# unanan/UNet_Nested4Tiny_Objects_Keypoints

Hardware: AMD Instinct MI355X
Metric: images/sec (train step) UNet++ L=4 256x256 (higher is better)
Workload: dtype f32

## Files before the change

include/unetpp_hip.h:

```cpp
#ifndef UNETPP_HIP_H
#define UNETPP_HIP_H

#include <stdint.h>

#ifdef __cplusplus
extern "C" {
#endif

#define UNETPP_ABI_VERSION 12
#define UNETPP_MAX_VIEWS 8

#define UNETPP_OK 0
#define UNETPP_EINVAL (-1)
#define UNETPP_ELAUNCH (-2)

typedef struct unetpp_view {
  float* ptr;
  int32_t C, c_off, c_len;
  int32_t Hs, Ws;
  int32_t sy, sx, oy, ox;
  const float* scale;
  const float* shift;
  const float* gate;
  int32_t relu;
// ... 207 lines not shown
                         float* out_nchw, void* stream);
int unetpp_head_bwd_bf16(const float* d_out_nchw, const float* out_nchw, const void* x, const float* weight,
                         int32_t N, int32_t H, int32_t W, int32_t C, int32_t n_cls, float p_drop, uint64_t seed,
                         const uint8_t* mask, const uint64_t* seed_dev, void* dx, int32_t accumulate, int32_t gate_x, float* partial,
                         void* stream);

int unetpp_maxpool_bwd_bf16(const void* d_pooled, const uint8_t* pool_idx, int32_t N, int32_t H, int32_t W, int32_t C,
                            void* d_act, const void* gate, void* stream);
int unetpp_bilinear2x_fwd_bf16(const void* x, int32_t N, int32_t H, int32_t W, int32_t C, void* y, void* stream);
int unetpp_bilinear2x_bwd_bf16(const void* dy, int32_t N, int32_t H, int32_t W, int32_t C, void* dx, int32_t accumulate,
                               const void* gate, void* stream);

int unetpp_first_layer_dgrad_bf16(const void* dy, const float* weight, int32_t N, int32_t H, int32_t W, int32_t CIN,
                                  int32_t COUT, float* dx, void* stream);

int64_t unetpp_heatmap_pattern_workspace_bytes(int32_t N, int32_t n_maps, int32_t H, int32_t W);
int unetpp_heatmap_pattern(const float* points, int32_t N, int32_t P, const int32_t* map_points,
                           const int32_t* map_begin, int32_t n_maps, int32_t H, int32_t W, float radius,
                           float* out_nchw, void* workspace, void* stream);
int64_t unetpp_keypoints_workspace_bytes(int32_t maps, int32_t H, int32_t W, int32_t max_regions);
int unetpp_keypoints_extract(int32_t stage, const float* heat, int32_t maps, int32_t H, int32_t W,
                             const float* thr_per_map, int32_t num, int32_t max_regions, int32_t sweeps,
                             void* workspace, int32_t* changed, float* points, int32_t* counts, void* stream);

#define UNETPP_OPTIM_ADAMW 0
#define UNETPP_OPTIM_ADABOUND 1
#define UNETPP_OPTIM_SGDW 2
#define UNETPP_OPTIM_AMS 1
#define UNETPP_OPTIM_CAPTURABLE 2
#define UNETPP_OPTIM_HYPER 8
// ... 125 lines not shown
```

unet_nested4tiny_objects_keypoints_amd/_lib.py:

```python
from __future__ import annotations

import ctypes as C
import os
import subprocess

_PKG_DIR = os.path.dirname(os.path.abspath(__file__))
_REPO = os.path.dirname(_PKG_DIR)
LIB_PATH = os.environ.get("UNETPP_LIB", os.path.join(_PKG_DIR, "libunetpp_hip.so"))
CSRC = os.path.join(_PKG_DIR, "csrc")
INCLUDE = os.path.join(_REPO, "include")
SOURCES = ("gemm_pix.hip", "gemm_fast.hip", "gemm_pw.hip", "gemm_pw_bf16.hip", "gemm_wino.hip", "gemm_bf16.hip", "gemm_bf16_dma.hip", "wgrad_bf16.hip", "pointwise_bf16.hip", "keypoints.hip", "weight_image.hip", "wgrad.hip", "wgrad_fast.hip", "wgrad_dma.hip", "wgrad_pw.hip", "wgrad_wino.hip", "first_layer.hip", "pointwise.hip", "caller.hip", "optim.hip", "validate.hip", "average.hip", "loader.hip", "scene.hip",
           "detect.hip", "crops.hip", "topk_loss.hip")
HEADERS = ("common.h", "gemm_units.h", "wgrad_reduce.h", "lds_asm.h", "bf16_common.h", "dropout.h", "bn_fused.h",
           "wino_experiments.h", "dma_experiments.h", "heads_mean.h", "focal_element.h")
MAX_VIEWS = 8
ABI_VERSION = 12
EXTRA_FLAGS = {"gemm_wino.hip": ("-fno-slp-vectorize",), "wgrad_wino.hip": ("-fno-slp-vectorize",)}
GEMM_DIRECT = 1
GEMM_BF16 = 2


class View(C.Structure):
    _fields_ = [
        ("ptr", C.c_void_p),
        ("C", C.c_int32), ("c_off", C.c_int32), ("c_len", C.c_int32),
        ("Hs", C.c_int32), ("Ws", C.c_int32),
        ("sy", C.c_int32), ("sx", C.c_int32), ("oy", C.c_int32), ("ox", C.c_int32),
        ("scale", C.c_void_p), ("shift", C.c_void_p), ("gate", C.c_void_p),
        ("relu", C.c_int32), ("accumulate", C.c_int32), ("gate_sum", C.c_int32), ("reserved", C.c_int32),
    ]


class BnFused(C.Structure):
    _fields_ = [
# ... 199 lines not shown
    "unetpp_optim_step_clip": (C.c_int, [_I32, _I32, _P, _I32, _P, _I64, _P, _P, _P, _P, _P, _P]),
    "unetpp_grad_scale": (C.c_int, [_P, _I32, _P, _I64, _P, _F, _P, _P]),
    "unetpp_warp_batch": (C.c_int, [_P, _I32, _I64, _I32, _I32, _I32, _P, _I32, _P, _P, _P, _F, _P, _I32, _I32, _P, _I32,
                                    _P, _P, _P]),
    "unetpp_augment_draw": (C.c_int, [_P, _I32, _U64, _I32, _I32, _I32, _I32, C.POINTER(AugmentDesc), _P]),
    "unetpp_scene_stitch": (C.c_int, [_P, _I32, _I32, _I32, _I32, _I32, C.POINTER(C.c_int32), C.POINTER(SceneRect), _P, _P,
                                      _I32, _I32, _I32, _P]),
    "unetpp_peaks_workspace_bytes": (_I64, [_I32, _I32, _I32]),
    "unetpp_peaks_detect": (C.c_int, [_P, _I32, _I32, _I32, _F, _I32, _I32, _I32, _P, _P, _P, _P, _P]),
    "unetpp_detect_match": (C.c_int, [_P, _P, _P, _I32, _I32, _I32, _P, _P, _I32, _F, _P, _P, _P, _P]),
    "unetpp_points_target": (C.c_int, [_P, _P, _I64, _I32, _P, _I32, _P, _I32, _I32, _I32, _F, _P, _P]),
    "unetpp_crops_draw": (C.c_int, [_P, _P, _P, _I32, _U64, _I32, _I32, _I32, _I32, _I32, _P, _P, _I32, _F, _F, _F,
                                    C.POINTER(AugmentDesc), _P]),
    "unetpp_topk_focal_workspace_bytes": (_I64, [_I32, _I64, _I64]),
    "unetpp_topk_focal_heads": (C.c_int, [C.POINTER(FocalHeads), _P, _I64, _I64, _I64, _I64, _F, _P, _P, _P, _P]),
}

_LIB = None


def source_hash() -> str:
    import hashlib
    h = hashlib.sha256()
    for path in [os.path.join(CSRC, s) for s in SOURCES + HEADERS] + [os.path.join(INCLUDE, "unetpp_hip.h")]:
        with open(path, "rb") as f:
            h.update(f.read())
    return h.hexdigest()[:16]


def build_library(force: bool = False, verbose: bool = False, out_path: str = None, obj_dir: str = None) -> str:
# ... 75 lines not shown
```

unet_nested4tiny_objects_keypoints_amd/csrc/common.h:

```cpp
#pragma once
#include <hip/hip_runtime.h>
#include <stdint.h>

#include "unetpp_hip.h"

typedef float f32x16 __attribute__((ext_vector_type(16)));
typedef float f32x4 __attribute__((ext_vector_type(4)));

namespace unetpp {

constexpr int kBlockPixels = 256;
constexpr int kThreads = 256;
constexpr int kMaxHaloPixels = 340;

struct TileGeom {
  int log2tw, tiles_x, tiles_y;
};

inline TileGeom tile_geom(int H, int W) {
  int l = 3;
  while ((1 << l) < W && l < 5) ++l;
  TileGeom g;
  g.log2tw = l;
  const int TW = 1 << l, TH = kBlockPixels >> l;
// ... 104 lines not shown
  OPT_BF16_DMA_MIN8,
  OPT_BF16_DMA_FORM,
  OPT_BF16_DMA_SMALL,
  OPT_BF16_DMA_STATS,
  OPT_BF16_DMA_POINTWISE,
  OPT_BF16_DMA_SPLIT,
  OPT_BF16_WGRAD_QUAD,
  OPT_WINO_NO_LEAN,
  OPT_WINO_ONE_PER_CU,
  OPT_MEMSET_NODES,
  OPT_BF16_PW_PLAIN,
  OPT_PW_DIRECT,
  OPT_PW_NT,
  OPT_HEAD_WGS_PER_CU,
  OPT_SMALL_WGRAD_BLOCKS,
  OPT_COUNT
};
bool opt_is_set(Opt o);
long opt_value(Opt o, long dflt);

int launch_gemm_fast(const unetpp_gemm_desc* d, hipStream_t st);
int launch_gemm_pw(const unetpp_gemm_desc* d, const struct FastArgs& fa, hipStream_t st);
int launch_gemm_pw_bf16(const unetpp_gemm_desc* d, const struct FastArgs& fa, hipStream_t st);
bool wino_applies(const unetpp_gemm_desc* d);
int launch_gemm_wino(const unetpp_gemm_desc* d, hipStream_t st, long* bn_rows);
bool bf16_gemm_args(const unetpp_gemm_desc* d, struct FastArgs& a);
int launch_gemm_bf16(const unetpp_gemm_desc* d, hipStream_t st);
int launch_gemm_bf16_dma(const unetpp_gemm_desc* d, hipStream_t st);
enum WgradKernel {
  WGRAD_FIRST_LAYER, WGRAD_BF16_QUAD, WGRAD_BF16_PAIR, WGRAD_PW, WGRAD_WINO, WGRAD_DMA, WGRAD_FAST, WGRAD_GENERIC
// ... 30 lines not shown
```

unet_nested4tiny_objects_keypoints_amd/csrc/first_layer.hip:

```cpp
#include "bf16_common.h"
#include "bn_fused.h"
#include "common.h"
#include "lds_asm.h"

namespace unetpp {
namespace {

constexpr int kMaxCout = 128;

struct SmallArgs {
  const float* x;
  const float* w;
  const float* bias;
  float* y;
  const float* dy;
  float* stats;
  float* slabs;
  int N, H, W, COUT, yC, relu;
  int log2tw, tiles_x, tiles_y;
  long n_patches;
  int bn_in_kernel;
};

template <int CIN>
__device__ __forceinline__ void stage_patch(const SmallArgs& a, float* xs, int n, int ty0, int tx0, int TW, int TH) {
  const int HWp = TW + 2, npix = HWp * (TH + 2);
  for (int it = threadIdx.x; it < npix * CIN; it += kThreads) {
    const int hp = it / CIN, ci = it - hp * CIN;
    const int hy = hp / HWp, hx = hp - hy * HWp;
    const int y = ty0 + hy - 1, x = tx0 + hx - 1;
    float v = 0.f;
    if (y >= 0 && y < a.H && x >= 0 && x < a.W) v = a.x[((static_cast<long>(n) * a.H + y) * a.W + x) * CIN + ci];
    xs[it] = v;
  }
}

template <int CIN, bool BF = false>
__global__ __launch_bounds__(kThreads, CIN >= 3 ? 3 : 4) void small_cin_fwd_kernel(const SmallArgs a) {
  constexpr int ITEMS = (kMaxHaloPixels * CIN + kThreads - 1) / kThreads;
  constexpr bool WREG = CIN <= 3;
  __shared__ float xs2[2][kMaxHaloPixels * CIN];
  __shared__ __attribute__((aligned(16))) float ws[WREG ? 4 : 9 * CIN * kMaxCout];
  __shared__ float red[4][kMaxCout * 2];
  const int tid = threadIdx.x;
  const bool bn_fused = a.bn_in_kernel != 0;
  float run1 = 0.f, run2 = 0.f;
  const int TW = 1 << a.log2tw, TH = kBlockPixels >> a.log2tw, HWp = TW + 2;
  const int npix = HWp * (TH + 2);
  const int QN = a.COUT >> 2;
// ... 46 lines not shown
    if (patch + gridDim.x < n_patches) request(patch + gridDim.x);

    unsigned b = patch;
    const int txi = static_cast<int>(b % static_cast<unsigned>(a.tiles_x));
    b /= static_cast<unsigned>(a.tiles_x);
    const int tyi = static_cast<int>(b % static_cast<unsigned>(a.tiles_y));
    const int n = static_cast<int>(b / static_cast<unsigned>(a.tiles_y));
    const int ty0 = tyi * TH, tx0 = txi * TW;
    float* y_patch = BF ? reinterpret_cast<float*>(reinterpret_cast<bf16_t*>(a.y) + ((static_cast<long>(n) * a.H + ty0) * a.W + tx0) * a.yC)
                        : a.y + ((static_cast<long>(n) * a.H + ty0) * a.W + tx0) * a.yC;
    f32x2_t s1a = {0.f, 0.f}, s1b = {0.f, 0.f}, s2a = {0.f, 0.f}, s2b = {0.f, 0.f};
    for (int p = psub; p < kBlockPixels; p += pstep) {
      const int py = p >> a.log2tw, px = p & (TW - 1);
      const int y = ty0 + py, x = tx0 + px;
      if (y < a.H && x < a.W) {
        f32x2_t acc_a = {bias4[0], bias4[1]}, acc_b = {bias4[2], bias4[3]};
#pragma unroll
        for (int tap = 0; tap < 9; ++tap) {
          const float* xp = &xs[((py + tap / 3) * HWp + px + tap % 3) * CIN];
#pragma unroll
          for (int ci = 0; ci < CIN; ++ci) {
            const f32x2_t xv = {xp[ci], xp[ci]};
            const f32x4 w4 = WREG ? wr[WREG ? tap * CIN + ci : 0]
                                  : *reinterpret_cast<const f32x4*>(&ws[WREG ? 0 : (tap * CIN + ci) * a.COUT + 4 * quad]);
            acc_a = __builtin_elementwise_fma(xv, f32x2_t{w4[0], w4[1]}, acc_a);
            acc_b = __builtin_elementwise_fma(xv, f32x2_t{w4[2], w4[3]}, acc_b);
          }
        }
        f32x4 acc = {acc_a.x, acc_a.y, acc_b.x, acc_b.y};
        if (a.relu) {
#pragma unroll
          for (int e = 0; e < 4; ++e) acc[e] = fmaxf(acc[e], 0.f);
        }
        if (BF) {
#pragma unroll
          for (int e = 0; e < 4; ++e) acc[e] = bf_round(acc[e]);
        }
        const f32x2_t va = {acc[0], acc[1]}, vb = {acc[2], acc[3]};
        s1a += va;
        s1b += vb;
        s2a = __builtin_elementwise_fma(va, va, s2a);
        s2b = __builtin_elementwise_fma(vb, vb, s2b);
        const unsigned o = static_cast<unsigned>((py * a.W + px) * a.yC + 4 * quad);
#ifndef UNETPP_FIRST_NO_NT
// ... 42 lines not shown
      }
    }
  }
  if (bn_fused) {
    __syncthreads();
    float* run = &red[0][0];
    if (tid < a.COUT) {
      run[2 * tid] = run1;
      run[2 * tid + 1] = run2;
    }
    __syncthreads();
    bn_rows_store<kThreads>(a.stats, a.COUT, run);
  }
}

template <int CIN, bool BF = false>
__global__ __launch_bounds__(kThreads) void small_cin_wgrad_kernel(const SmallArgs a) {
  __shared__ float xs[kMaxHaloPixels * CIN];
  __shared__ float red[kThreads][4];
  const int tid = threadIdx.x;
  const int TW = 1 << a.log2tw, TH = kBlockPixels >> a.log2tw, HWp = TW + 2;
  const int QN = a.COUT >> 2;
  const int quad = tid % QN, psub = tid / QN, pstep = kThreads / QN;
  f32x4 acc[9 * CIN];
#pragma unroll
  for (int i = 0; i < 9 * CIN; ++i) acc[i] = f32x4{0.f, 0.f, 0.f, 0.f};
  f32x4 db = {0.f, 0.f, 0.f, 0.f};
  for (long patch = blockIdx.x; patch < a.n_patches; patch += gridDim.x) {
    long b = patch;
    const int txi = static_cast<int>(b % a.tiles_x);
// ... 32 lines not shown
#pragma unroll
        for (int e = 0; e < 4; ++e) db[e] += g[e];
#pragma unroll
        for (int tap = 0; tap < 9; ++tap) {
          const float* xp = &xs[((py + tap / 3) * HWp + px + tap % 3) * CIN];
#pragma unroll
          for (int ci = 0; ci < CIN; ++ci) {
            const float xv = xp[ci];
#pragma unroll
            for (int e = 0; e < 4; ++e) acc[tap * CIN + ci][e] = fmaf(xv, g[e], acc[tap * CIN + ci][e]);
          }
        }
      }
    }
  }
  float* slab = a.slabs + static_cast<long>(blockIdx.x) * (9 * CIN + 1) * a.COUT;
#pragma unroll
  for (int row = 0; row <= 9 * CIN; ++row) {
    const f32x4 v = (row < 9 * CIN) ? acc[row < 9 * CIN ? row : 0] : db;
    __syncthreads();
#pragma unroll
    for (int e = 0; e < 4; ++e) red[tid][e] = v[e];
    __syncthreads();
    for (int c = tid; c < a.COUT; c += kThreads) {
      const int q = c >> 2, e = c & 3;
      float t = 0.f;
      for (int k = q; k < kThreads; k += QN) t += red[k][e];
      slab[row * a.COUT + c] = t;
    }
  }
}

template <int CIN>
__global__ __launch_bounds__(kThreads) void small_cin_dgrad_bf16_kernel(const bf16_t* __restrict__ dy,
                                                                        const float* __restrict__ w, int N, int H, int W,
                                                                        int COUT, float* __restrict__ dx) {
  __shared__ float ws[9 * kMaxCout * CIN];
  for (int i = threadIdx.x; i < 9 * COUT * CIN; i += kThreads) {
    const int ci = i % CIN, co = (i / CIN) % COUT, tap = i / (CIN * COUT);
    ws[i] = w[(static_cast<long>(co) * CIN + ci) * 9 + tap];
  }
  __syncthreads();
  const long pixels = static_cast<long>(N) * H * W;
  for (long p = blockIdx.x * static_cast<long>(kThreads) + threadIdx.x; p < pixels; p += static_cast<long>(gridDim.x) * kThreads) {
    const int x = static_cast<int>(p % W);
// ... 136 lines not shown
  if (reinterpret_cast<uintptr_t>(dy) & 15) return UNETPP_EINVAL;
  const long pixels = static_cast<long>(N) * H * W;
  long blocks = (pixels + kThreads - 1) / kThreads;
  if (blocks > 4096) blocks = 4096;
  const dim3 grid(static_cast<unsigned>(blocks)), block(kThreads);
  hipStream_t st = static_cast<hipStream_t>(stream);
  const bf16_t* g = static_cast<const bf16_t*>(dy);
  switch (CIN) {
    case 1: hipLaunchKernelGGL(small_cin_dgrad_bf16_kernel<1>, grid, block, 0, st, g, weight, N, H, W, COUT, dx); break;
    case 2: hipLaunchKernelGGL(small_cin_dgrad_bf16_kernel<2>, grid, block, 0, st, g, weight, N, H, W, COUT, dx); break;
    case 3: hipLaunchKernelGGL(small_cin_dgrad_bf16_kernel<3>, grid, block, 0, st, g, weight, N, H, W, COUT, dx); break;
    default: hipLaunchKernelGGL(small_cin_dgrad_bf16_kernel<4>, grid, block, 0, st, g, weight, N, H, W, COUT, dx); break;
  }
  return launch_status();
}
```

unet_nested4tiny_objects_keypoints_amd/csrc/gemm_pix.hip:

```cpp
#include "bn_fused.h"
#include <atomic>
#include <cstdio>
#include <cstdlib>
#include <cstring>
#include <mutex>

#include "common.h"
#include "gemm_units.h"

namespace unetpp {
namespace {

constexpr int KC = 16;
constexpr int KCP = 20;
constexpr int WJ = 12;

struct GemmArgs {
  unetpp_gemm_desc d;
  int log2tw, tiles_x, tiles_y;
  int Ktot, Ncols;
};

template <int TAPS>
__global__ __launch_bounds__(kThreads, 2) void gemm_pix_kernel(const GemmArgs a) {
// ... 138 lines not shown
      dst[1] = t2;
    }
  }
}

}
}

namespace unetpp {
namespace {
thread_local const char* g_last_kernel = "";

const char* const kOptNames[OPT_COUNT] = {
    "BF16_NO_DMA", "BF16_DMA_ALL", "BF16_DMA_MIN8", "BF16_DMA_FORM", "BF16_DMA_SMALL", "BF16_DMA_STATS",
    "BF16_DMA_POINTWISE", "BF16_DMA_SPLIT", "BF16_WGRAD_QUAD", "WINO_NO_LEAN", "WINO_ONE_PER_CU", "MEMSET_NODES",
    "BF16_PW_PLAIN", "PW_DIRECT", "PW_NT", "HEAD_WGS_PER_CU", "SMALL_WGRAD_BLOCKS"};
struct OptSlot {
  std::atomic<long> value{0};
  std::atomic<bool> set{false};
};
OptSlot g_opts[OPT_COUNT];
std::atomic<int> g_reserved_cus{0};
std::once_flag g_opts_once;

void opts_from_environment() {
  std::call_once(g_opts_once, [] {
    char name[64];
    for (int i = 0; i < OPT_COUNT; ++i) {
      snprintf(name, sizeof(name), "UNETPP_%s", kOptNames[i]);
      const char* e = getenv(name);
      if (e != nullptr) {
// ... 167 lines not shown
```

unet_nested4tiny_objects_keypoints_amd/engine.py:

```python
from __future__ import annotations

import os

from typing import Dict, List, Optional, Tuple

import torch

from . import ops
from .ops import V


USE_PACK_PLAN = os.environ.get("UNETPP_NO_PACK_PLAN") is None
USE_GROUPED_DGRAD = os.environ.get("UNETPP_NO_GROUPED_DGRAD") is None
USE_PLAN_COPIES = os.environ.get("UNETPP_NO_PLAN_COPIES") is None
_A1_MATERIALIZE_BYTES = int(float(os.environ.get("UNETPP_BF16_A1_MAX_MB", "80")) * (1 << 20))
_A1_MATERIALIZE_BYTES_F32 = int(float(os.environ.get("UNETPP_F32_A1_MAX_MB", "80")) * (1 << 20))


def _empty(n, like):
    return torch.empty(n, dtype=torch.float32, device=like.device)


def _packed(w, t, k, n, dstr, sstr, flip=False):
    dst = _empty(t * k * n, w)
    ops.pack_weight(dst, w, t, k, n, dstr, sstr, flip=flip)
    return dst


# ... 39 lines not shown
        dst, ready = plan.copy_for(("bias4", b.data_ptr()) + ops.phase_tag(plan.phase), plan.phase, (b.data_ptr(), co),
                                   lambda: (_empty(4 * co, b), [b], [(b, 0, 0, 4, co, 0, co)]))
        if ready:
            return dst
    else:
        dst = _empty(4 * co, b)
    ops.pack_weight(dst, b, 4, 1, co, (co, 0, 1), (0, 0, 1))
    return dst


def _phase_views(t, **kw):
    return [V(t, sy=2, sx=2, oy=a, ox=b, **kw) for a in (0, 1) for b in (0, 1)]


class _PairRec:
    __slots__ = ("ins", "y1", "a1", "y2", "out", "pooled", "pool_idx", "bn1", "bn2", "frozen1", "frozen2", "h", "w")

    def __init__(self):
        for s in self.__slots__:
            setattr(self, s, None)


class _UpRec:
    __slots__ = ("src", "up", "interp", "h", "w")

    def __init__(self):
        for s in self.__slots__:
            setattr(self, s, None)


class _Saved:
# ... 30 lines not shown
    conv1, conv2 = getattr(blk.conv1, "0"), getattr(blk.conv2, "0")
    co = conv1.out_channels
    like = ins[0].t
    new = lambda: torch.empty((b, h, w, co), dtype=adt, device=like.device)
    r = _PairRec()
    r.ins, r.h, r.w = ins, h, w
    if pool:
        r.pooled = torch.empty((b, h // 2, w // 2, co), dtype=adt, device=like.device)
        r.pool_idx = torch.empty((b, h // 2, w // 2, co), dtype=torch.uint8, device=like.device)
    if blk.is_batchnorm:
        bn1, bn2 = getattr(blk.conv1, "1"), getattr(blk.conv2, "1")
        t1, t2 = bool(getattr(bn1, "training", training)), bool(getattr(bn2, "training", training))
        r.frozen1, r.frozen2 = not t1, not t2
        r.y1 = new()
        r.bn1 = _conv_bn_fwd(ins, conv1, bn1, r.y1, b, h, w, t1, stats)
        r.y2 = new()
        if ((adt == torch.bfloat16 and r.y1.numel() * 2 <= _A1_MATERIALIZE_BYTES) or
                (adt == torch.float32 and r.y1.numel() * 4 <= _A1_MATERIALIZE_BYTES_F32)):
            r.a1 = new()
            ops.affine_relu_pool(r.y1, r.bn1[2], r.bn1[3], True, r.a1, None, None)
            r.bn2 = _conv_bn_fwd([V(r.a1)], conv2, bn2, r.y2, b, h, w, t2, stats)
        else:
            r.bn2 = _conv_bn_fwd([V(r.y1, scale=r.bn1[2], shift=r.bn1[3], relu=True)], conv2, bn2, r.y2, b, h, w, t2, stats)
        r.out = new()
        ops.affine_relu_pool(r.y2, r.bn2[2], r.bn2[3], True, r.out, r.pooled, r.pool_idx)
    else:
        r.a1 = new()
        ops.gemm_fwd(b, h, w, 9, ins, [V(r.a1, relu=True)], pack_conv_fwd(conv1.weight.detach()), conv1.bias.detach())
        r.out = new()
        ops.gemm_fwd(b, h, w, 9, [V(r.a1)], [V(r.out, relu=True)], pack_conv_fwd(conv2.weight.detach()),
# ... 275 lines not shown
    conv1, conv2 = getattr(blk.conv1, "0"), getattr(blk.conv2, "0")
    h, w = r.h, r.w
    if blk.is_batchnorm:
        bn1, bn2 = getattr(blk.conv1, "1"), getattr(blk.conv2, "1")
        grads[bn2.weight], grads[bn2.bias] = _bn_bwd(bn2, r.bn2, r.frozen2, d_out, r.y2, pool_grad)
        dy2 = V(d_out)
        mean, invstd, scale, shift = r.bn1
        if r.a1 is not None:
            _conv_wgrad(conv2, [V(r.a1)], [dy2], b, h, w, grads)
        else:
            _conv_wgrad(conv2, [V(r.y1, scale=scale, shift=shift, relu=True)], [dy2], b, h, w, grads)
        if flush is not None:
            flush()
        d_a1 = torch.empty_like(r.y1)
        ops.gemm_fwd(b, h, w, 9, [dy2], [V(d_a1)], pack_conv_dgrad(conv2.weight.detach()))
        grads[bn1.weight], grads[bn1.bias] = _bn_bwd(bn1, r.bn1, r.frozen1, d_a1, r.y1, None)
        dy1 = V(d_a1)
    else:
        dy2 = V(d_out) if pre_gated else V(d_out, gate=r.out)
        _conv_wgrad(conv2, [V(r.a1)], [dy2], b, h, w, grads)
        if flush is not None:
            flush()
        d_a1 = torch.empty_like(r.a1)
        ops.gemm_fwd(b, h, w, 9, [dy2], [V(d_a1, gate=r.a1)], pack_conv_dgrad(conv2.weight.detach()))
        dy1 = V(d_a1)
    _conv_wgrad(conv1, r.ins, [dy1], b, h, w, grads)
    if flush is not None:
        flush()
    if in_targets is not None:
        if dy1.t.dtype == torch.bfloat16 and in_targets[0].t.dtype == torch.float32:
# ... 207 lines not shown
```

unet_nested4tiny_objects_keypoints_amd/ops.py:

```python
from __future__ import annotations

import ctypes as C
import functools
import os
from dataclasses import dataclass
from typing import Optional, Sequence

import torch

from . import _lib
from ._lib import MAX_VIEWS, GemmDesc, PackJob, View, WeightSrc, WgradDesc, check


def _stream():
    return C.c_void_p(torch.cuda.current_stream().cuda_stream)


class LaunchTimer:

    def __init__(self):
        self.launches = []
        self.regions = []
        self.want_launches = True
        self.want_regions = True
# ... 305 lines not shown

_PLAN: Optional[PackPlan] = None


def set_pack_plan(plan: Optional[PackPlan]) -> None:
    global _PLAN
    _PLAN = plan


def current_plan() -> Optional[PackPlan]:
    return _PLAN if (_PLAN is not None and _PLAN.phase is not None) else None


def phase_tag(phase) -> tuple:
    return () if phase in ("fwd", "bwd") else (phase,)


def gemm_pixel_blocks(n: int, h: int, w: int) -> int:
    return int(_lib.lib().unetpp_gemm_pixel_blocks(n, h, w))


@dataclass
class BatchNormFinish:
    gamma: torch.Tensor
    beta: torch.Tensor
    running_mean: Optional[torch.Tensor]
    running_var: Optional[torch.Tensor]
    eps: float
    momentum: float
    count: int
# ... 213 lines not shown
                                       c, _ptr(partial), st), "unetpp_bn_bwd_reduce")
    else:
        d_pooled, pool_idx = _need(pool[0], "d_pooled"), _need(pool[1], "pool_idx", torch.uint8)
        check(lib.unetpp_bn_bwd_reduce_pool(_ptr(d_act), _ptr(y), _ptr(scale), _ptr(shift), _ptr(mean), _ptr(invstd),
                                            _ptr(d_pooled), _ptr(pool_idx), n, h, w, c, _ptr(partial), st),
              "unetpp_bn_bwd_reduce_pool")
    check(lib.unetpp_bn_bwd_finalize(_ptr(partial), blocks, c, _ptr(dgamma), _ptr(dbeta), st), "unetpp_bn_bwd_finalize")
    if pool is None:
        check(lib.unetpp_bn_bwd_apply(_ptr(d_act), _ptr(y), _ptr(scale), _ptr(shift), _ptr(mean), _ptr(invstd),
                                      _ptr(gamma), _ptr(dgamma), _ptr(dbeta), pixels, c, _ptr(dy_out), st),
              "unetpp_bn_bwd_apply")
    else:
        check(lib.unetpp_bn_bwd_apply_pool(_ptr(d_act), _ptr(y), _ptr(scale), _ptr(shift), _ptr(mean), _ptr(invstd),
                                           _ptr(gamma), _ptr(dgamma), _ptr(dbeta), _ptr(pool[0]), _ptr(pool[1]), n, h,
                                           w, c, _ptr(dy_out), st), "unetpp_bn_bwd_apply_pool")
    return dgamma, dbeta


def bn_frozen_backward(d_act, y, scale, shift, mean, invstd, dy_out, dgamma=None, dbeta=None, pool=None, want_sums=True):
    lib = _lib.lib()
    n, h, w, c = y.shape
    pixels = n * h * w
    bf16 = _is_bf16(y)
    adt = torch.bfloat16 if bf16 else torch.float32
    _need(d_act, "d_act", adt), _need(y, "y", adt), _need(dy_out, "dy", adt)
    if tuple(d_act.shape) != tuple(y.shape) or tuple(dy_out.shape) != tuple(y.shape):
        raise ValueError("d_act, y and dy must have one shape")
    if want_sums and (mean is None or invstd is None):
        raise ValueError("the gamma / beta sums need the running mean snapshot and invstd")
    blocks_fn = lib.unetpp_bn_frozen_bwd_blocks_bf16 if bf16 else lib.unetpp_bn_frozen_bwd_blocks
# ... 571 lines not shown
```

Measured before the change: 1712.

## Fuse first-layer BatchNorm backward into weight-gradient kernel with optional conv recompute

```diff
diff --git a/include/unetpp_hip.h b/include/unetpp_hip.h
--- a/include/unetpp_hip.h
+++ b/include/unetpp_hip.h
@@ -245,6 +245,20 @@
 int unetpp_first_layer_dgrad_bf16(const void* dy, const float* weight, int32_t N, int32_t H, int32_t W, int32_t CIN,
                                   int32_t COUT, float* dx, void* stream);
 
+#define UNETPP_FIRST_BN_BF16 1
+#define UNETPP_FIRST_BN_FROZEN 2
+#define UNETPP_FIRST_BN_WANT_DX 4
+#define UNETPP_FIRST_BN_UNALIGNED 8
+int unetpp_first_bn_bwd_ok(int32_t N, int32_t H, int32_t W, int32_t CIN, int32_t COUT, int32_t flags);
+int unetpp_first_bn_recomputes(int32_t CIN);
+int unetpp_first_bn_reduce(const float* x, const float* weight, const float* bias, const float* d_act, const float* y,
+                           const float* scale, const float* shift, const float* mean, const float* invstd, int32_t N,
+                           int32_t H, int32_t W, int32_t CIN, int32_t COUT, int32_t n_rows, float* partial, void* stream);
+int unetpp_first_bn_wgrad(const float* x, const float* weight, const float* bias, const float* d_act, const float* y,
+                          const float* scale, const float* shift, const float* mean, const float* invstd,
+                          const float* gamma, const float* dgamma, const float* dbeta, int32_t N, int32_t H, int32_t W,
+                          int32_t CIN, int32_t COUT, int32_t n_split, float* slabs, void* stream);
+
 int64_t unetpp_heatmap_pattern_workspace_bytes(int32_t N, int32_t n_maps, int32_t H, int32_t W);
 int unetpp_heatmap_pattern(const float* points, int32_t N, int32_t P, const int32_t* map_points,
                            const int32_t* map_begin, int32_t n_maps, int32_t H, int32_t W, float radius,
diff --git a/unet_nested4tiny_objects_keypoints_amd/_lib.py b/unet_nested4tiny_objects_keypoints_amd/_lib.py
--- a/unet_nested4tiny_objects_keypoints_amd/_lib.py
+++ b/unet_nested4tiny_objects_keypoints_amd/_lib.py
@@ -18,6 +18,7 @@
 EXTRA_FLAGS = {"gemm_wino.hip": ("-fno-slp-vectorize",), "wgrad_wino.hip": ("-fno-slp-vectorize",)}
 GEMM_DIRECT = 1
 GEMM_BF16 = 2
+FIRST_BN_BF16, FIRST_BN_FROZEN, FIRST_BN_WANT_DX, FIRST_BN_UNALIGNED = 1, 2, 4, 8
 
 
 class View(C.Structure):
@@ -247,6 +248,10 @@
                                     C.POINTER(AugmentDesc), _P]),
     "unetpp_topk_focal_workspace_bytes": (_I64, [_I32, _I64, _I64]),
     "unetpp_topk_focal_heads": (C.c_int, [C.POINTER(FocalHeads), _P, _I64, _I64, _I64, _I64, _F, _P, _P, _P, _P]),
+    "unetpp_first_bn_bwd_ok": (C.c_int, [_I32, _I32, _I32, _I32, _I32, _I32]),
+    "unetpp_first_bn_recomputes": (C.c_int, [_I32]),
+    "unetpp_first_bn_reduce": (C.c_int, [_P] * 9 + [_I32] * 6 + [_P, _P]),
+    "unetpp_first_bn_wgrad": (C.c_int, [_P] * 12 + [_I32] * 6 + [_P, _P]),
 }
 
 _LIB = None
diff --git a/unet_nested4tiny_objects_keypoints_amd/csrc/common.h b/unet_nested4tiny_objects_keypoints_amd/csrc/common.h
--- a/unet_nested4tiny_objects_keypoints_amd/csrc/common.h
+++ b/unet_nested4tiny_objects_keypoints_amd/csrc/common.h
@@ -142,6 +142,7 @@
   OPT_PW_NT,
   OPT_HEAD_WGS_PER_CU,
   OPT_SMALL_WGRAD_BLOCKS,
+  OPT_FIRST_BN_RECOMPUTE,
   OPT_COUNT
 };
 bool opt_is_set(Opt o);
diff --git a/unet_nested4tiny_objects_keypoints_amd/csrc/first_layer.hip b/unet_nested4tiny_objects_keypoints_amd/csrc/first_layer.hip
--- a/unet_nested4tiny_objects_keypoints_amd/csrc/first_layer.hip
+++ b/unet_nested4tiny_objects_keypoints_amd/csrc/first_layer.hip
@@ -22,8 +22,8 @@
   int bn_in_kernel;
 };
 
-template <int CIN>
-__device__ __forceinline__ void stage_patch(const SmallArgs& a, float* xs, int n, int ty0, int tx0, int TW, int TH) {
+template <int CIN, typename Args>
+__device__ __forceinline__ void stage_patch(const Args& a, float* xs, int n, int ty0, int tx0, int TW, int TH) {
   const int HWp = TW + 2, npix = HWp * (TH + 2);
   for (int it = threadIdx.x; it < npix * CIN; it += kThreads) {
     const int hp = it / CIN, ci = it - hp * CIN;
@@ -33,6 +33,23 @@
     if (y >= 0 && y < a.H && x >= 0 && x < a.W) v = a.x[((static_cast<long>(n) * a.H + y) * a.W + x) * CIN + ci];
     xs[it] = v;
   }
+}
+
+template <int CIN, typename WAt>
+__device__ __forceinline__ f32x4 conv_quad(const float* xs, int py, int px, int HWp, const f32x4 bias4, WAt w_at) {
+  f32x2_t acc_a = {bias4[0], bias4[1]}, acc_b = {bias4[2], bias4[3]};
+#pragma unroll
+  for (int tap = 0; tap < 9; ++tap) {
+    const float* xp = &xs[((py + tap / 3) * HWp + px + tap % 3) * CIN];
+#pragma unroll
+    for (int ci = 0; ci < CIN; ++ci) {
+      const f32x2_t xv = {xp[ci], xp[ci]};
+      const f32x4 w4 = w_at(tap * CIN + ci);
+      acc_a = __builtin_elementwise_fma(xv, f32x2_t{w4[0], w4[1]}, acc_a);
+      acc_b = __builtin_elementwise_fma(xv, f32x2_t{w4[2], w4[3]}, acc_b);
+    }
+  }
+  return f32x4{acc_a.x, acc_a.y, acc_b.x, acc_b.y};
 }
 
 template <int CIN, bool BF = false>
@@ -109,20 +126,9 @@
       const int py = p >> a.log2tw, px = p & (TW - 1);
       const int y = ty0 + py, x = tx0 + px;
       if (y < a.H && x < a.W) {
-        f32x2_t acc_a = {bias4[0], bias4[1]}, acc_b = {bias4[2], bias4[3]};
-#pragma unroll
-        for (int tap = 0; tap < 9; ++tap) {
-          const float* xp = &xs[((py + tap / 3) * HWp + px + tap % 3) * CIN];
-#pragma unroll
-          for (int ci = 0; ci < CIN; ++ci) {
-            const f32x2_t xv = {xp[ci], xp[ci]};
-            const f32x4 w4 = WREG ? wr[WREG ? tap * CIN + ci : 0]
-                                  : *reinterpret_cast<const f32x4*>(&ws[WREG ? 0 : (tap * CIN + ci) * a.COUT + 4 * quad]);
-            acc_a = __builtin_elementwise_fma(xv, f32x2_t{w4[0], w4[1]}, acc_a);
-            acc_b = __builtin_elementwise_fma(xv, f32x2_t{w4[2], w4[3]}, acc_b);
-          }
-        }
-        f32x4 acc = {acc_a.x, acc_a.y, acc_b.x, acc_b.y};
+        f32x4 acc = conv_quad<CIN>(xs, py, px, HWp, bias4, [&](int t) {
+          return WREG ? wr[WREG ? t : 0] : *reinterpret_cast<const f32x4*>(&ws[WREG ? 0 : t * a.COUT + 4 * quad]);
+        });
         if (a.relu) {
 #pragma unroll
           for (int e = 0; e < 4; ++e) acc[e] = fmaxf(acc[e], 0.f);
@@ -195,6 +201,25 @@
   }
 }
 
+template <int CIN>
+__device__ __forceinline__ void store_slab(const f32x4 (&acc)[9 * CIN], const f32x4 db, float (*red)[4], float* slab, int COUT) {
+  const int tid = threadIdx.x, QN = COUT >> 2;
+#pragma unroll
+  for (int row = 0; row <= 9 * CIN; ++row) {
+    const f32x4 v = (row < 9 * CIN) ? acc[row < 9 * CIN ? row : 0] : db;
+    __syncthreads();
+#pragma unroll
+    for (int e = 0; e < 4; ++e) red[tid][e] = v[e];
+    __syncthreads();
+    for (int c = tid; c < COUT; c += kThreads) {
+      const int q = c >> 2, e = c & 3;
+      float t = 0.f;
+      for (int k = q; k < kThreads; k += QN) t += red[k][e];
+      slab[row * COUT + c] = t;
+    }
+  }
+}
+
 template <int CIN, bool BF = false>
 __global__ __launch_bounds__(kThreads) void small_cin_wgrad_kernel(const SmallArgs a) {
   __shared__ float xs[kMaxHaloPixels * CIN];
@@ -257,21 +282,212 @@
       }
     }
   }
-  float* slab = a.slabs + static_cast<long>(blockIdx.x) * (9 * CIN + 1) * a.COUT;
-#pragma unroll
-  for (int row = 0; row <= 9 * CIN; ++row) {
-    const f32x4 v = (row < 9 * CIN) ? acc[row < 9 * CIN ? row : 0] : db;
-    __syncthreads();
-#pragma unroll
-    for (int e = 0; e < 4; ++e) red[tid][e] = v[e];
-    __syncthreads();
-    for (int c = tid; c < a.COUT; c += kThreads) {
-      const int q = c >> 2, e = c & 3;
-      float t = 0.f;
-      for (int k = q; k < kThreads; k += QN) t += red[k][e];
-      slab[row * a.COUT + c] = t;
-    }
-  }
+  store_slab<CIN>(acc, db, red, a.slabs + static_cast<long>(blockIdx.x) * (9 * CIN + 1) * a.COUT, a.COUT);
+}
+
+struct FirstBnArgs {
+  const float* x;
+  const float* w;
+  const float* bias;
+  const float* g;
+  const float* y;
+  const float *scale, *shift, *mean, *invstd;
+  const float *gamma, *dgamma, *dbeta;
+  float inv_count;
+  float* out;
+  int N, H, W, COUT;
+  int log2tw, tiles_x, tiles_y;
+  long n_patches;
+};
+
+__device__ __forceinline__ f32x4 quad_of(const float* p, int quad) {
+  return f32x4{p[4 * quad], p[4 * quad + 1], p[4 * quad + 2], p[4 * quad + 3]};
+}
+
+template <int CIN>
+__device__ __forceinline__ void first_bn_weights(const FirstBnArgs& a, int quad, f32x4* wr, float* ws) {
+  if (CIN == 1) {
+#pragma unroll
+    for (int tap = 0; tap < 9; ++tap)
+#pragma unroll
+      for (int e = 0; e < 4; ++e) wr[tap][e] = a.w[(4 * quad + e) * 9 + tap];
+  } else {
+    for (int i = threadIdx.x; i < 9 * CIN * a.COUT; i += kThreads) {
+      const int co = i % a.COUT, t = i / a.COUT, tap = t / CIN, ci = t - tap * CIN;
+      ws[i] = a.w[(co * CIN + ci) * 9 + tap];
+    }
+  }
+}
+
+template <int G, bool RECOMPUTE>
+__device__ __forceinline__ unsigned first_bn_load(const FirstBnArgs& a, int n, int ty0, int tx0, int p0, int pstep, int quad,
+                                                  f32x4 (&gq)[G], f32x4 (&yq)[RECOMPUTE ? 1 : G]) {
+  const int TW = 1 << a.log2tw;
+  unsigned live = 0;
+#pragma unroll
+  for (int u = 0; u < G; ++u) {
+    const int p = p0 + u * pstep;
+    const int py = p >> a.log2tw, px = p & (TW - 1);
+    const int y = ty0 + py, x = tx0 + px;
+    const bool ok = (p < kBlockPixels) & (y < a.H) & (x < a.W);
+    const long o = ((static_cast<long>(n) * a.H + (ok ? y : ty0)) * a.W + (ok ? x : tx0)) * a.COUT + 4 * quad;
+    const f32x4 g = *reinterpret_cast<const f32x4*>(a.g + o);
+#pragma unroll
+    for (int e = 0; e < 4; ++e) gq[u][e] = ok ? g[e] : 0.f;
+    if (!RECOMPUTE) yq[RECOMPUTE ? 0 : u] = *reinterpret_cast<const f32x4*>(a.y + o);
+    live |= (ok ? 1u : 0u) << u;
+  }
+  return live;
+}
+
+template <int CIN, bool RECOMPUTE>
+__global__ __launch_bounds__(kThreads) void first_bn_reduce_kernel(const FirstBnArgs a) {
+  constexpr bool WREG = CIN == 1;
+  constexpr int G = 8;
+  __shared__ float xs[RECOMPUTE ? kMaxHaloPixels * CIN : 1];
+  __shared__ __attribute__((aligned(16))) float ws[(RECOMPUTE && !WREG) ? 9 * CIN * kMaxCout : 4];
+  __shared__ float red[kThreads][8];
+  const int tid = threadIdx.x;
+  const int TW = 1 << a.log2tw, TH = kBlockPixels >> a.log2tw, HWp = TW + 2;
+  const int QN = a.COUT >> 2;
+  const int quad = tid % QN, psub = tid / QN, pstep = kThreads / QN;
+  f32x4 wr[(RECOMPUTE && WREG) ? 9 : 1];
+  f32x4 bias4 = {0.f, 0.f, 0.f, 0.f};
+  if (RECOMPUTE) {
+    first_bn_weights<CIN>(a, quad, wr, ws);
+    if (a.bias != nullptr) bias4 = quad_of(a.bias, quad);
+  }
+  const f32x4 sc = quad_of(a.scale, quad), sh = quad_of(a.shift, quad), mu = quad_of(a.mean, quad), is = quad_of(a.invstd, quad);
+  f32x4 s1 = {0.f, 0.f, 0.f, 0.f}, s2 = {0.f, 0.f, 0.f, 0.f};
+  for (long patch = blockIdx.x; patch < a.n_patches; patch += gridDim.x) {
+    long b = patch;
+    const int txi = static_cast<int>(b % a.tiles_x);
+    b /= a.tiles_x;
+    const int tyi = static_cast<int>(b % a.tiles_y);
+    const int n = static_cast<int>(b / a.tiles_y);
+    const int ty0 = tyi * TH, tx0 = txi * TW;
+    if (RECOMPUTE) {
+      __syncthreads();
+      stage_patch<CIN>(a, xs, n, ty0, tx0, TW, TH);
+      __syncthreads();
+    }
+    for (int p0 = psub; p0 < kBlockPixels; p0 += G * pstep) {
+      f32x4 gq[G], yq[RECOMPUTE ? 1 : G];
+      first_bn_load<G, RECOMPUTE>(a, n, ty0, tx0, p0, pstep, quad, gq, yq);
+#pragma unroll
+      for (int u = 0; u < G; ++u) {
+        const int p = min(p0 + u * pstep, kBlockPixels - 1);
+        const int py = p >> a.log2tw, px = p & (TW - 1);
+        f32x4 yv;
+        if (RECOMPUTE)
+          yv = conv_quad<CIN>(xs, py, px, HWp, bias4, [&](int t) {
+            return WREG ? wr[(RECOMPUTE && WREG) ? t : 0] : *reinterpret_cast<const f32x4*>(&ws[(RECOMPUTE && !WREG) ? t * a.COUT + 4 * quad : 0]);
+          });
+        else
+          yv = yq[RECOMPUTE ? 0 : u];
+#pragma unroll
+        for (int e = 0; e < 4; ++e) {
+          const float gg = (fmaf(yv[e], sc[e], sh[e]) > 0.f) ? gq[u][e] : 0.f;
+          s1[e] += gg;
+          s2[e] = fmaf(gg * (yv[e] - mu[e]), is[e], s2[e]);
+        }
+      }
+    }
+  }
+#pragma unroll
+  for (int e = 0; e < 4; ++e) {
+    red[tid][e] = s1[e];
+    red[tid][4 + e] = s2[e];
+  }
+  __syncthreads();
+  if (tid < a.COUT) {
+    const int q = tid >> 2, e = tid & 3;
+    double t1 = 0.0, t2 = 0.0;
+    for (int k = q; k < kThreads; k += QN) {
+      t1 += static_cast<double>(red[k][e]);
+      t2 += static_cast<double>(red[k][4 + e]);
+    }
+    float* dst = a.out + (static_cast<long>(blockIdx.x) * a.COUT + tid) * 2;
+    dst[0] = static_cast<float>(t1);
+    dst[1] = static_cast<float>(t2);
+  }
+}
+
+template <int CIN, bool RECOMPUTE>
+__global__ __launch_bounds__(kThreads, CIN == 1 ? 2 : 1) void first_bn_wgrad_kernel(const FirstBnArgs a) {
+  constexpr bool WREG = CIN == 1;
+  constexpr int G = RECOMPUTE ? (CIN == 1 ? 4 : 2) : (CIN >= 3 ? 4 : 8);
+  __shared__ float xs[kMaxHaloPixels * CIN];
+  __shared__ __attribute__((aligned(16))) float ws[(RECOMPUTE && !WREG) ? 9 * CIN * kMaxCout : 4];
+  __shared__ float red[kThreads][4];
+  const int tid = threadIdx.x;
+  const int TW = 1 << a.log2tw, TH = kBlockPixels >> a.log2tw, HWp = TW + 2;
+  const int QN = a.COUT >> 2;
+  const int quad = tid % QN, psub = tid / QN, pstep = kThreads / QN;
+  f32x4 wr[(RECOMPUTE && WREG) ? 9 : 1];
+  f32x4 bias4 = {0.f, 0.f, 0.f, 0.f};
+  if (RECOMPUTE) {
+    first_bn_weights<CIN>(a, quad, wr, ws);
+    if (a.bias != nullptr) bias4 = quad_of(a.bias, quad);
+  }
+  const f32x4 sc = quad_of(a.scale, quad), sh = quad_of(a.shift, quad), mu = quad_of(a.mean, quad), is = quad_of(a.invstd, quad);
+  const f32x4 dgam = quad_of(a.dgamma, quad), dbet = quad_of(a.dbeta, quad);
+  const f32x4 k4 = quad_of(a.gamma, quad) * is;
+  const float neg_inv = -a.inv_count;
+  f32x4 acc[9 * CIN];
+#pragma unroll
+  for (int i = 0; i < 9 * CIN; ++i) acc[i] = f32x4{0.f, 0.f, 0.f, 0.f};
+  f32x4 db = {0.f, 0.f, 0.f, 0.f};
+  for (long patch = blockIdx.x; patch < a.n_patches; patch += gridDim.x) {
+    long b = patch;
+    const int txi = static_cast<int>(b % a.tiles_x);
+    b /= a.tiles_x;
+    const int tyi = static_cast<int>(b % a.tiles_y);
+    const int n = static_cast<int>(b / a.tiles_y);
+    const int ty0 = tyi * TH, tx0 = txi * TW;
+    __syncthreads();
+    stage_patch<CIN>(a, xs, n, ty0, tx0, TW, TH);
+    __syncthreads();
+    for (int p0 = psub; p0 < kBlockPixels; p0 += G * pstep) {
+      f32x4 gq[G], yq[RECOMPUTE ? 1 : G];
+      const unsigned live = first_bn_load<G, RECOMPUTE>(a, n, ty0, tx0, p0, pstep, quad, gq, yq);
+#pragma unroll
+      for (int u = 0; u < G; ++u) {
+        const int p = min(p0 + u * pstep, kBlockPixels - 1);
+        const int py = p >> a.log2tw, px = p & (TW - 1);
+        f32x4 yv;
+        if (RECOMPUTE)
+          yv = conv_quad<CIN>(xs, py, px, HWp, bias4, [&](int t) {
+            return WREG ? wr[(RECOMPUTE && WREG) ? t : 0] : *reinterpret_cast<const f32x4*>(&ws[(RECOMPUTE && !WREG) ? t * a.COUT + 4 * quad : 0]);
+          });
+        else
+          yv = yq[RECOMPUTE ? 0 : u];
+        f32x4 g;
+#pragma unroll
+        for (int e = 0; e < 4; ++e) {
+          const float gg = (fmaf(yv[e], sc[e], sh[e]) > 0.f) ? gq[u][e] : 0.f;
+          const float xhat = (yv[e] - mu[e]) * is[e];
+          float t = fmaf(neg_inv, dbet[e], gg);
+          t = fmaf(neg_inv, xhat * dgam[e], t);
+          g[e] = ((live >> u) & 1u) ? k4[e] * t : 0.f;
+        }
+#pragma unroll
+        for (int e = 0; e < 4; ++e) db[e] += g[e];
+#pragma unroll
+        for (int tap = 0; tap < 9; ++tap) {
+          const float* xp = &xs[((py + tap / 3) * HWp + px + tap % 3) * CIN];
+#pragma unroll
+          for (int ci = 0; ci < CIN; ++ci) {
+            const float xv = xp[ci];
+#pragma unroll
+            for (int e = 0; e < 4; ++e) acc[tap * CIN + ci][e] = fmaf(xv, g[e], acc[tap * CIN + ci][e]);
+          }
+        }
+        if (RECOMPUTE) __builtin_amdgcn_sched_barrier(0);
+      }
+    }
+  }
+  store_slab<CIN>(acc, db, red, a.out + static_cast<long>(blockIdx.x) * (9 * CIN + 1) * a.COUT, a.COUT);
 }
 
 template <int CIN>
@@ -438,3 +654,115 @@
   }
   return launch_status();
 }
+
+namespace unetpp {
+namespace {
+bool first_bn_recomputes(int CIN) {
+  const long v = opt_value(OPT_FIRST_BN_RECOMPUTE, -1);
+  return v < 0 ? CIN == 1 : v != 0;
+}
+
+bool first_bn_shape_ok(int N, int H, int W, int CIN, int COUT) {
+  if (N < 1 || H < 1 || W < 1 || CIN < 1 || CIN > 4) return false;
+  if (COUT < 4 || (COUT & 3) || COUT > kMaxCout || (kThreads % (COUT >> 2)) != 0) return false;
+  return static_cast<long>(N) * H * W * COUT < 0x80000000L;
+}
+
+struct FirstBnCall {
+  const float *x, *weight, *bias, *d_act, *y, *scale, *shift, *mean, *invstd;
+  int N, H, W, CIN, COUT, rows;
+};
+
+int first_bn_args(const FirstBnCall& c, FirstBnArgs& a) {
+  if (!c.x || !c.d_act || !c.y || !c.scale || !c.shift || !c.mean || !c.invstd) return UNETPP_EINVAL;
+  if (!first_bn_shape_ok(c.N, c.H, c.W, c.CIN, c.COUT)) return UNETPP_EINVAL;
+  if ((reinterpret_cast<uintptr_t>(c.d_act) | reinterpret_cast<uintptr_t>(c.y)) & 15) return UNETPP_EINVAL;
+  const TileGeom g = tile_geom(c.H, c.W);
+  a = FirstBnArgs{};
+  a.n_patches = static_cast<long>(c.N) * g.tiles_y * g.tiles_x;
+  if (c.rows < 1 || c.rows > a.n_patches || c.rows > 4096) return UNETPP_EINVAL;
+  a.x = c.x;
+  a.w = c.weight;
+  a.bias = c.bias;
+  a.g = c.d_act;
+  a.y = c.y;
+  a.scale = c.scale;
+  a.shift = c.shift;
+  a.mean = c.mean;
+  a.invstd = c.invstd;
+  a.N = c.N;
+  a.H = c.H;
+  a.W = c.W;
+  a.COUT = c.COUT;
+  a.log2tw = g.log2tw;
+  a.tiles_x = g.tiles_x;
+  a.tiles_y = g.tiles_y;
+  return UNETPP_OK;
+}
+
+#define UNETPP_FIRST_BN_LAUNCH(KERNEL, CIN, RC, grid, st, a)                                            \
+  switch (CIN) {                                                                                        \
+    case 1: hipLaunchKernelGGL((KERNEL<1, RC>), grid, dim3(kThreads), 0, st, a); break;                 \
+    case 2: hipLaunchKernelGGL((KERNEL<2, RC>), grid, dim3(kThreads), 0, st, a); break;                 \
+    case 3: hipLaunchKernelGGL((KERNEL<3, RC>), grid, dim3(kThreads), 0, st, a); break;                 \
+    default: hipLaunchKernelGGL((KERNEL<4, RC>), grid, dim3(kThreads), 0, st, a); break;                \
+  }
+}
+}
+
+extern "C" int unetpp_first_bn_bwd_ok(int32_t N, int32_t H, int32_t W, int32_t CIN, int32_t COUT, int32_t flags) {
+  return (flags == 0 && unetpp::first_bn_shape_ok(N, H, W, CIN, COUT)) ? 1 : 0;
+}
+
+extern "C" int unetpp_first_bn_recomputes(int32_t CIN) {
+  return (CIN >= 1 && CIN <= 4 && unetpp::first_bn_recomputes(CIN)) ? 1 : 0;
+}
+
+extern "C" int unetpp_first_bn_reduce(const float* x, const float* weight, const float* bias, const float* d_act,
+                                      const float* y, const float* scale, const float* shift, const float* mean,
+                                      const float* invstd, int32_t N, int32_t H, int32_t W, int32_t CIN, int32_t COUT,
+                                      int32_t n_rows, float* partial, void* stream) {
+  using namespace unetpp;
+  if (partial == nullptr || (reinterpret_cast<uintptr_t>(partial) & 7)) return UNETPP_EINVAL;
+  const bool rc = weight != nullptr && CIN >= 1 && CIN <= 4 && first_bn_recomputes(CIN);
+  FirstBnArgs a;
+  const FirstBnCall c = {x, weight, bias, d_act, y, scale, shift, mean, invstd, N, H, W, CIN, COUT, n_rows};
+  if (first_bn_args(c, a) != UNETPP_OK) return UNETPP_EINVAL;
+  a.out = partial;
+  const dim3 grid(static_cast<unsigned>(n_rows));
+  hipStream_t st = static_cast<hipStream_t>(stream);
+  note_kernel(rc ? "first_bn_reduce_kernel/recompute" : "first_bn_reduce_kernel/read");
+  if (rc) {
+    UNETPP_FIRST_BN_LAUNCH(first_bn_reduce_kernel, CIN, true, grid, st, a)
+  } else {
+    UNETPP_FIRST_BN_LAUNCH(first_bn_reduce_kernel, CIN, false, grid, st, a)
+  }
+  return launch_status();
+}
+
+extern "C" int unetpp_first_bn_wgrad(const float* x, const float* weight, const float* bias, const float* d_act,
+                                     const float* y, const float* scale, const float* shift, const float* mean,
+                                     const float* invstd, const float* gamma, const float* dgamma, const float* dbeta,
+                                     int32_t N, int32_t H, int32_t W, int32_t CIN, int32_t COUT, int32_t n_split,
+                                     float* slabs, void* stream) {
+  using namespace unetpp;
+  if (!gamma || !dgamma || !dbeta || !slabs) return UNETPP_EINVAL;
+  const bool rc = weight != nullptr && CIN >= 1 && CIN <= 4 && first_bn_recomputes(CIN);
+  FirstBnArgs a;
+  const FirstBnCall c = {x, weight, bias, d_act, y, scale, shift, mean, invstd, N, H, W, CIN, COUT, n_split};
+  if (first_bn_args(c, a) != UNETPP_OK) return UNETPP_EINVAL;
+  a.gamma = gamma;
+  a.dgamma = dgamma;
+  a.dbeta = dbeta;
+  a.inv_count = 1.0f / static_cast<float>(static_cast<long>(N) * H * W);
+  a.out = slabs;
+  const dim3 grid(static_cast<unsigned>(n_split));
+  hipStream_t st = static_cast<hipStream_t>(stream);
+  note_kernel(rc ? "first_bn_wgrad_kernel/recompute" : "first_bn_wgrad_kernel/read");
+  if (rc) {
+    UNETPP_FIRST_BN_LAUNCH(first_bn_wgrad_kernel, CIN, true, grid, st, a)
+  } else {
+    UNETPP_FIRST_BN_LAUNCH(first_bn_wgrad_kernel, CIN, false, grid, st, a)
+  }
+  return launch_status();
+}
diff --git a/unet_nested4tiny_objects_keypoints_amd/csrc/gemm_pix.hip b/unet_nested4tiny_objects_keypoints_amd/csrc/gemm_pix.hip
--- a/unet_nested4tiny_objects_keypoints_amd/csrc/gemm_pix.hip
+++ b/unet_nested4tiny_objects_keypoints_amd/csrc/gemm_pix.hip
@@ -176,7 +176,7 @@
 const char* const kOptNames[OPT_COUNT] = {
     "BF16_NO_DMA", "BF16_DMA_ALL", "BF16_DMA_MIN8", "BF16_DMA_FORM", "BF16_DMA_SMALL", "BF16_DMA_STATS",
     "BF16_DMA_POINTWISE", "BF16_DMA_SPLIT", "BF16_WGRAD_QUAD", "WINO_NO_LEAN", "WINO_ONE_PER_CU", "MEMSET_NODES",
-    "BF16_PW_PLAIN", "PW_DIRECT", "PW_NT", "HEAD_WGS_PER_CU", "SMALL_WGRAD_BLOCKS"};
+    "BF16_PW_PLAIN", "PW_DIRECT", "PW_NT", "HEAD_WGS_PER_CU", "SMALL_WGRAD_BLOCKS", "FIRST_BN_RECOMPUTE"};
 struct OptSlot {
   std::atomic<long> value{0};
   std::atomic<bool> set{false};
diff --git a/unet_nested4tiny_objects_keypoints_amd/engine.py b/unet_nested4tiny_objects_keypoints_amd/engine.py
--- a/unet_nested4tiny_objects_keypoints_amd/engine.py
+++ b/unet_nested4tiny_objects_keypoints_amd/engine.py
@@ -12,6 +12,8 @@
 
 USE_PACK_PLAN = os.environ.get("UNETPP_NO_PACK_PLAN") is None
 USE_GROUPED_DGRAD = os.environ.get("UNETPP_NO_GROUPED_DGRAD") is None
+USE_FIRST_BN_BWD = os.environ.get("UNETPP_NO_FIRST_BN_BWD") is None
+_FIRST_BN_BWD_CIN = (1, 4)
 USE_PLAN_COPIES = os.environ.get("UNETPP_NO_PLAN_COPIES") is None
 _A1_MATERIALIZE_BYTES = int(float(os.environ.get("UNETPP_BF16_A1_MAX_MB", "80")) * (1 << 20))
 _A1_MATERIALIZE_BYTES_F32 = int(float(os.environ.get("UNETPP_F32_A1_MAX_MB", "80")) * (1 << 20))
@@ -81,7 +83,8 @@
 
 
 class _PairRec:
-    __slots__ = ("ins", "y1", "a1", "y2", "out", "pooled", "pool_idx", "bn1", "bn2", "frozen1", "frozen2", "h", "w")
+    __slots__ = ("ins", "y1", "a1", "y2", "out", "pooled", "pool_idx", "bn1", "bn2", "frozen1", "frozen2", "h", "w",
+                 "y1_small_cin")
 
     def __init__(self):
         for s in self.__slots__:
@@ -142,6 +145,7 @@
         r.frozen1, r.frozen2 = not t1, not t2
         r.y1 = new()
         r.bn1 = _conv_bn_fwd(ins, conv1, bn1, r.y1, b, h, w, t1, stats)
+        r.y1_small_cin = len(ins) == 1 and ins[0].t.shape[3] <= 4 and ops.last_kernel() == "small_cin_fwd_kernel"
         r.y2 = new()
         if ((adt == torch.bfloat16 and r.y1.numel() * 2 <= _A1_MATERIALIZE_BYTES) or
                 (adt == torch.float32 and r.y1.numel() * 4 <= _A1_MATERIALIZE_BYTES_F32)):
@@ -447,6 +451,20 @@
             flush()
         d_a1 = torch.empty_like(r.y1)
         ops.gemm_fwd(b, h, w, 9, [dy2], [V(d_a1)], pack_conv_dgrad(conv2.weight.detach()))
+        x_in = r.ins[0]
+        if (USE_FIRST_BN_BWD and in_targets is None and len(r.ins) == 1 and x_in.t.shape[3] in _FIRST_BN_BWD_CIN
+                and (x_in.c_off, x_in.sy, x_in.sx, x_in.oy, x_in.ox) == (0, 1, 1, 0, 0) and x_in.c_len is None
+                and x_in.scale is None and x_in.gate is None and not x_in.relu
+                and ops.first_bn_bwd_ok(x_in.t, d_a1, r.y1, frozen=r.frozen1)):
+            dgamma, dbeta = _new_grad(bn1.weight), _new_grad(bn1.bias)
+            dw, db = _new_grad(conv1.weight), _new_grad(conv1.bias)
+            ops.first_bn_backward(x_in.t, conv1.weight.detach(), conv1.bias.detach(), d_a1, r.y1, scale, shift, mean,
+                                  invstd, bn1.weight.detach(), dgamma, dbeta, dw, db, recompute_ok=bool(r.y1_small_cin))
+            grads[bn1.weight], grads[bn1.bias] = dgamma, dbeta
+            grads[conv1.weight], grads[conv1.bias] = dw, db
+            if flush is not None:
+                flush()
+            return None
         grads[bn1.weight], grads[bn1.bias] = _bn_bwd(bn1, r.bn1, r.frozen1, d_a1, r.y1, None)
         dy1 = V(d_a1)
     else:
diff --git a/unet_nested4tiny_objects_keypoints_amd/ops.py b/unet_nested4tiny_objects_keypoints_amd/ops.py
--- a/unet_nested4tiny_objects_keypoints_amd/ops.py
+++ b/unet_nested4tiny_objects_keypoints_amd/ops.py
@@ -343,6 +343,10 @@
 
 def phase_tag(phase) -> tuple:
     return () if phase in ("fwd", "bwd") else (phase,)
+
+
+def last_kernel() -> str:
+    return _lib.lib().unetpp_last_kernel_name().decode()
 
 
 def gemm_pixel_blocks(n: int, h: int, w: int) -> int:
@@ -586,6 +590,67 @@
         check(lib.unetpp_bn_bwd_apply_pool(_ptr(d_act), _ptr(y), _ptr(scale), _ptr(shift), _ptr(mean), _ptr(invstd),
                                            _ptr(gamma), _ptr(dgamma), _ptr(dbeta), _ptr(pool[0]), _ptr(pool[1]), n, h,
                                            w, c, _ptr(dy_out), st), "unetpp_bn_bwd_apply_pool")
+    return dgamma, dbeta
+
+
+def first_bn_bwd_ok(x, d_act, y, frozen=False, want_input_grad=False) -> bool:
+    if x.dim() != 4 or y.dim() != 4 or tuple(d_act.shape) != tuple(y.shape) or tuple(x.shape[:3]) != tuple(y.shape[:3]):
+        return False
+    flags = 0
+    if y.dtype != torch.float32 or d_act.dtype != torch.float32 or x.dtype != torch.float32:
+        flags |= _lib.FIRST_BN_BF16
+    if frozen:
+        flags |= _lib.FIRST_BN_FROZEN
+    if want_input_grad:
+        flags |= _lib.FIRST_BN_WANT_DX
+    if not (x.is_contiguous() and y.is_contiguous() and d_act.is_contiguous()) or (y.data_ptr() | d_act.data_ptr()) % 16:
+        flags |= _lib.FIRST_BN_UNALIGNED
+    n, h, w, c = y.shape
+    return bool(_lib.lib().unetpp_first_bn_bwd_ok(n, h, w, x.shape[3], c, flags))
+
+
+def first_bn_backward(x, weight, bias, d_act, y, scale, shift, mean, invstd, gamma, dgamma, dbeta, dw, db,
+                      recompute_ok=True):
+    lib = _lib.lib()
+    n, h, w, c = y.shape
+    cin = x.shape[3]
+    for t, what in ((x, "x"), (d_act, "d_act"), (y, "y"), (weight, "weight"), (scale, "scale"), (shift, "shift"),
+                    (mean, "mean"), (invstd, "invstd"), (gamma, "gamma"), (dgamma, "dgamma"), (dbeta, "dbeta"),
+                    (dw, "dw"), (db, "db")):
+        _need(t, what)
+    if bias is not None:
+        _need(bias, "bias")
+    if tuple(weight.shape) != (c, cin, 3, 3) or tuple(dw.shape) != (c, cin, 3, 3) or db.numel() != c:
+        raise ValueError("shape mismatch")
+    d = WgradDesc()
+    d.N, d.H, d.W, d.taps, d.n_x, d.n_dy = n, h, w, 9, 1, 1
+    V(x).fill(d.x[0])
+    V(d_act).fill(d.dy[0])
+    plan = _lib.WgradSizes()
+    check(lib.unetpp_wgrad_plan(C.byref(d), 0, C.byref(plan)), "unetpp_wgrad_plan")
+    split = plan.n_split
+    if plan.planes != 9 or plan.slab_floats != split * (9 * cin + 1) * c:
+        raise RuntimeError("first_bn_backward: the weight-gradient plan is not the first layer's (%s)" % plan.kernel)
+    partial = torch.empty(split * c * 2, dtype=torch.float32, device=y.device)
+    slabs = torch.empty(plan.slab_floats, dtype=torch.float32, device=y.device)
+    st = _stream()
+    tensor_bytes = 4.0 * n * h * w * c
+    w_arg, b_arg = (weight, bias) if recompute_ok else (None, None)
+    y_bytes = 0.0 if (recompute_ok and lib.unetpp_first_bn_recomputes(cin)) else tensor_bytes
+    _timed_call(None, 0.0,
+                lambda: check(lib.unetpp_first_bn_reduce(_ptr(x), _ptr(w_arg), _ptr(b_arg), _ptr(d_act), _ptr(y), _ptr(scale),
+                                                         _ptr(shift), _ptr(mean), _ptr(invstd), n, h, w, cin, c, split,
+                                                         _ptr(partial), st), "unetpp_first_bn_reduce"),
+                tensor_bytes + y_bytes + 4.0 * n * h * w * cin)
+    check(lib.unetpp_bn_bwd_finalize(_ptr(partial), split, c, _ptr(dgamma), _ptr(dbeta), st), "unetpp_bn_bwd_finalize")
+    _timed_call(None, 2.0 * n * h * w * 9 * cin * c,
+                lambda: check(lib.unetpp_first_bn_wgrad(_ptr(x), _ptr(w_arg), _ptr(b_arg), _ptr(d_act), _ptr(y), _ptr(scale),
+                                                        _ptr(shift), _ptr(mean), _ptr(invstd), _ptr(gamma), _ptr(dgamma),
+                                                        _ptr(dbeta), n, h, w, cin, c, split, _ptr(slabs), st),
+                              "unetpp_first_bn_wgrad"),
+                tensor_bytes + y_bytes + 4.0 * n * h * w * cin)
+    check(lib.unetpp_wgrad_finish(_ptr(slabs), split, 9, cin, c, c, _ptr(dw), 1, 9, cin * 9, 0, _ptr(db), st),
+          "unetpp_wgrad_finish")
     return dgamma, dbeta
 
 
```

Result: no change. 1727 (median of 6 runs) (+0.9%).
